# Xinjie-Q/Boosting-NeRV

Hardware: AMD Instinct MI355X
Metric: train frames/sec (higher is better)
Workload: dtype fp32; 1 GPU; NeRV-boost 1.5M (1489577 params, fc_dim 30) train step on a synthetic Bunny-shaped clip 132x3x720x1280: decoder fwd + Fusion10_freq + bwd + fused Adan; frames resident in HBM; global_batch=1, per_gpu_batch=1, parallelism=dp1, hipgraph=True, rccl_ranks=0, collective_in_graph=False

## Files before the change

### boosting_nerv_amd/csrc/abi.hip

```cpp
#include "common.h"
#include <string.h>

namespace { thread_local char g_err[512] = ""; }

int bnerv_set_error(int code, const char* fmt, ...) {
    va_list ap;
    va_start(ap, fmt);
    vsnprintf(g_err, sizeof(g_err), fmt, ap);
    va_end(ap);
    return code;
}

extern "C" int bnerv_abi_version(void) { return BNERV_ABI_VERSION; }
extern "C" const char* bnerv_last_error(void) { return g_err; }
extern "C" const char* bnerv_build_arch(void) { return "gfx950"; }

#include "sidejob.h"
#include <new>
#include <vector>

namespace {
__global__ __launch_bounds__(256) void side_flush_kernel(const SidePack sp) {
    __shared__ float red[256];
    side_slice<SidePack, true>(sp, blockIdx.x, red);
// ... 11 lines not shown
    j.out = out;
    j.out2 = out2;
    j.n_slabs = n_slabs;
    j.count = count;
    j.ncols = ncols;
    int lanes = 8;
    while (lanes < 128 && lanes * 16 < n_slabs) lanes *= 2;
    j.epb = 256 / lanes;
    j.slices = (count + j.epb - 1) / j.epb;
    return j;
}
}

void bnerv_side_push(bnerv_ctx* ctx, hipStream_t st, const void* src, int n_slabs, int count, int ncols, float* out, float* out2, const float* fold_scale, const float* fold_shift) {
    const SideJob j = make_job(src, n_slabs, count, ncols, out, out2, fold_scale, fold_shift);
    if (ctx) { ctx->queue.push_back(j); return; }
    SidePack sp;
    sp.j[0] = j;
    sp.n_jobs = 1;
    sp.n_slices = j.slices;
    hipLaunchKernelGGL(side_flush_kernel, dim3(sp.n_slices), dim3(256), 0, st, sp);
}

void bnerv_side_take(bnerv_ctx* ctx, SidePack* sp, int max_slices) {
    sp->n_jobs = 0;
    sp->n_slices = 0;
    if (!ctx) return;
    std::vector<SideJob>& q = ctx->queue;
    int n = 0;
    size_t i = 0;
    while (i < q.size() && n < SIDE_MAX_JOBS) {
        if (q[i].fs) { ++i; continue; }
        if (sp->n_slices + q[i].slices > max_slices) break;
        sp->j[n] = q[i];
        sp->n_slices += q[i].slices;
        ++n;
        q.erase(q.begin() + (long)i);
    }
    sp->n_jobs = n;
}

int bnerv_side_pending(const bnerv_ctx* ctx) { return ctx ? (int)ctx->queue.size() : 0; }

int bnerv_side_flush(bnerv_ctx* ctx, hipStream_t st) {
    while (ctx && !ctx->queue.empty()) {
        SideFlushPack sp;
        std::vector<SideJob>& q = ctx->queue;
        int n = 0;
        sp.n_slices = 0;
        while (n < (int)q.size() && n < SIDE_FLUSH_JOBS) {
            sp.j[n] = q[n];
            sp.start[n] = sp.n_slices;
            sp.n_slices += q[n].slices;
            ++n;
        }
        for (int k = n; k < SIDE_FLUSH_JOBS; ++k) sp.start[k] = 0x7fffffff;
// ... 57 lines not shown
```

### boosting_nerv_amd/csrc/sidejob.h

```cpp
#pragma once
#include "common.h"

constexpr int SIDE_MAX_JOBS = 4;

struct SideJob {
    const float* src;
    float* out;
    float* out2;
    int n_slabs, count, ncols;
    int epb;
    int slices;
    const float* fs;
    const float* ft;
};

struct SidePack {
    SideJob j[SIDE_MAX_JOBS];
    int n_jobs, n_slices;
};
constexpr int SIDE_FLUSH_JOBS = 32;
struct SideFlushPack {
    SideJob j[SIDE_FLUSH_JOBS];
    int n_jobs, n_slices;
    int start[SIDE_FLUSH_JOBS];
};

#include <vector>
struct bnerv_ctx {
    std::vector<SideJob> queue;
    void* scratch = nullptr;
    size_t scratch_bytes = 0;
    struct BfWPlan* wplan = nullptr;
};
void bnerv_wplan_free(bnerv_ctx* ctx);
void* bnerv_ctx_scratch(bnerv_ctx* ctx, size_t bytes, hipStream_t st);

void bnerv_side_push(bnerv_ctx* ctx, hipStream_t st, const void* src, int n_slabs, int count, int ncols, float* out, float* out2,
                     const float* fold_scale = nullptr, const float* fold_shift = nullptr);
void bnerv_side_take(bnerv_ctx* ctx, SidePack* sp, int max_slices);
int bnerv_side_flush(bnerv_ctx* ctx, hipStream_t st);
int bnerv_side_pending(const bnerv_ctx* ctx);

template <class Pack>
__device__ __forceinline__ int side_find_job(const Pack& sp, int* s) {
    int j = 0;
    while (j < sp.n_jobs - 1 && *s >= sp.j[j].slices) { *s -= sp.j[j].slices; ++j; }
    return j;
}
template <>
__device__ __forceinline__ int side_find_job<SideFlushPack>(const SideFlushPack& sp, int* s) {
    const int k = (int)(threadIdx.x & 63);
    const int st = k < sp.n_jobs ? sp.start[k < SIDE_FLUSH_JOBS ? k : 0] : 0x7fffffff;
    const unsigned long long m = __ballot(st <= *s);
    const int j = __popcll(m) - 1;
    *s -= __shfl(st, j, 64);
    return __builtin_amdgcn_readfirstlane(j);
}

template <class Pack, bool FOLD = false>
__device__ __forceinline__ void side_slice(const Pack& sp, int s, float* red) {
    const int j = side_find_job(sp, &s);
    const SideJob& job = sp.j[j];
// ... 70 lines not shown
```

### boosting_nerv_amd/csrc/wgrad.hip

```cpp
#include "common.h"
#include "sidejob.h"
#include "split16.h"
#include "conv4_body.h"
#include "convs_body.h"
#if defined(BNERV_TRACE) || defined(BNERV_TRACE_BW)
static __device__ unsigned long long g_trace_w[1024 * 4 * 8 * 8];
#endif
#ifdef BNERV_TRACE_BW
#define BTRACE(it_, slot) do { if (lane == 0 && blockIdx.x < 1024 && (unsigned)(it_) < 8u) g_trace_w[((blockIdx.x * 4 + wave) * 8 + (it_)) * 8 + (slot)] = __builtin_amdgcn_s_memtime(); } while (0)
#endif
#include "wgrad_bfw_body.h"
#include "route.h"
bool bnerv_stem_wgrad_ok(const bnerv_wgrad_desc& d);
int bnerv_stem_wgrad_launch(hipStream_t st, const bnerv_wgrad_desc& d);
bool bnerv_stem_pair_ok(const bnerv_conv_desc& c, const bnerv_wgrad_desc& d);
int bnerv_stem_pair_launch(hipStream_t st, const bnerv_conv_desc& c, const bnerv_wgrad_desc& d);
int bnerv_wgrad1x1_slabs(const bnerv_wgrad_desc& d);
int bnerv_wgrad1x1_launch(hipStream_t st, const bnerv_wgrad_desc& d);

namespace {
using namespace bnerv_wb;

constexpr int TH = 8, TW = 32;
constexpr int CSG = TH * TW + 2;
// ... 546 lines not shown

    int bbase[NTW];
#pragma unroll
    for (int nt = 0; nt < NTW; ++nt) {
        const int n = nt * 16 + li;
        int off;
        if (n < nW) {
            const int ci = n / G::T, tap = n - ci * G::T;
            off = ci * G::PLANE + (tap / KS) * G::RS + (tap % KS) + G::COL0;
        } else {
            off = (n == nW ? NPLL : NPLL + 1) * G::PLANE;
        }
        bbase[nt] = off + (2 * wave) * G::RS + kq;
    }
    const int abase = li * CSG + wave * 64 + kq;

    f32x4 acc[NTW];
#pragma unroll
    for (int n = 0; n < NTW; ++n) acc[n] = f32x4{0.f, 0.f, 0.f, 0.f};
    int aff_b = -1;
    if (has_work) {
        issue(it);
        if constexpr (AFF) { load_affine(it.b); aff_b = it.b; }
        commit(it);
    }
    WTRACE(7, 1);
    int wt = 0; (void)wt;
    for (; itx < r1; itx += nlb, ++wt) {
        WTRACE(wt, 0);
        const bool has_next = itx + nlb < r1;
        LTile nxt = it;
        if (has_next) nxt = advance(it);
        lds_barrier();
        WTRACE(wt, 1);
        const Pre pre = prep(nxt);
        WTRACE(wt, 2);
#pragma unroll
        for (int st = 0; st < 16; ++st) {
            if (has_next) {
#pragma unroll
                for (int p = 0; p < NPART; ++p)
                    if (p * 16 / NPART == st) issue_part(pre, p);
            }
            float bf[NTW];
            const float af = s_g[abase + st * 4];
#pragma unroll
            for (int n = 0; n < NTW; ++n) bf[n] = s_in[bbase[n] + ((st >> 3) * G::RS + (st & 7) * 4)];
#pragma unroll
            for (int n = 0; n < NTW; ++n) acc[n] = __builtin_amdgcn_mfma_f32_16x16x4f32(af, bf[n], acc[n], 0, 0, 0);
        }
        WTRACE(wt, 3);
        lds_barrier();
        WTRACE(wt, 5);
        if (has_next) {
            if constexpr (AFF) { if (nxt.b != aff_b) { load_affine(nxt.b); aff_b = nxt.b; } }
            commit(nxt);
        }
        WTRACE(wt, 6);
        it = nxt;
    }
    WTRACE(7, 2);

    __syncthreads();
    float* s_red = smem;
    constexpr int RW = NTW * 16, RSZ = 16 * RW;
#pragma unroll
    for (int n = 0; n < NTW; ++n)
#pragma unroll
        for (int r = 0; r < 4; ++r) s_red[wave * RSZ + (4 * kq + r) * RW + n * 16 + li] = acc[n][r];
    __syncthreads();
    float* slab = wa.slab + (size_t)vb * Cout * wa.ncols;
    for (int idx = tid; idx < RSZ; idx += 256) {
        const int row = idx / RW, col = idx - row * RW;
        if (row < Cout && col < wa.ncols)
            slab[(size_t)row * wa.ncols + col] = (s_red[idx] + s_red[RSZ + idx]) + (s_red[2 * RSZ + idx] + s_red[3 * RSZ + idx]);
    }
    WTRACE(7, 3);
    side_run_hosted(side, smem, vb, vgrid);
    WTRACE(7, 4);
}
template <int KS, int IN, int GM2>
__global__ __launch_bounds__(256, (KS == 3 ? 3 : 4)) void wgrad_lean_kernel(const WArgs wa, const int n_grows, const SidePack side) {
    wgrad_lean_body<KS, IN, GM2>(wa, n_grows, side, (int)blockIdx.x, (int)gridDim.x);
}
template <int EP, int WIN>
__global__ __launch_bounds__(256, 3) void conv_wgrad_pair_kernel(const bnerv_conv::KArgs ka, const WArgs wa, const int n_grows, const int n_conv, const SidePack side, const int pat) {
    if (n_conv < 0) {
        const int nr = -n_conv, xcd = (int)blockIdx.x & 7, slot = (int)blockIdx.x >> 3, vb = ((slot >> 1) << 3) + xcd;
        const int role = pat == 0 ? (slot & 1) : ((slot + (slot >> pat)) & 1);
        if (role == 0) {
            SidePack none;
            none.n_jobs = 0; none.n_slices = 0;
            bnerv_q4::conv_q4_body<BNERV_IN_PLAIN, EP>(ka, none, vb, nr);
        } else {
            wgrad_lean_body<3, WIN, 0>(wa, n_grows, side, vb, nr);
        }
        return;
    }
    if ((int)blockIdx.x < n_conv) {
        SidePack none;
        none.n_jobs = 0; none.n_slices = 0;
        bnerv_q4::conv_q4_body<BNERV_IN_PLAIN, EP>(ka, none, (int)blockIdx.x, n_conv);
    } else {
        wgrad_lean_body<3, WIN, 0>(wa, n_grows, side, (int)blockIdx.x - n_conv, (int)gridDim.x - n_conv);
    }
}

#include "pairf_body.h"
template <int EP, int WIN>
__global__ __launch_bounds__(256, 2) void pair_fused_kernel(const bnerv_conv::KArgs ka, const WArgs wa, const SidePack side) {
    pair_fused_body<EP, WIN>(ka, wa, side, (int)blockIdx.x, (int)gridDim.x);
}
template <int EP>
__global__ __launch_bounds__(256, 2) void pair_fold_kernel(const bnerv_conv::KArgs ka, const WArgs wa, const SidePack side) {
    pair_fold_body<EP>(ka, wa, side, (int)blockIdx.x, (int)gridDim.x);
}

constexpr size_t WLEAN_MAX_BYTES = 0x7ff00000;

template <class F>
int wlean_modes(const bnerv_wgrad_desc& d, F&& f) {
    const int in = d.in_mode, gm = d.g_mode;
    if (gm == BNERV_IN_TANHGRAD && in == BNERV_IN_PLAIN) return f(mode_c<BNERV_IN_PLAIN>{}, mode_c<2>{});
    if (gm == BNERV_IN_PLAIN || gm == BNERV_IN_UNSHUFFLE) {
        const bool pair = gm == BNERV_IN_UNSHUFFLE && d.g_s == 2;
        if (in == BNERV_IN_PLAIN) return pair ? f(mode_c<BNERV_IN_PLAIN>{}, mode_c<1>{}) : f(mode_c<BNERV_IN_PLAIN>{}, mode_c<0>{});
        if (d.k == 3 && !pair && in == BNERV_IN_AFFINE) return f(mode_c<BNERV_IN_AFFINE>{}, mode_c<0>{});
// ... 31 lines not shown
    const size_t lds_red = (size_t)4 * 16 * NTW * 16;
    return (lds_main > lds_red ? lds_main : lds_red) * sizeof(float);
}

template <int KS, int IN, int GM2>
int launch_wlean(hipStream_t st, const WArgs& wa) {
    const int n_grows = wa.d.Cout <= 12 ? 12 : 16;
    const size_t lds = wlean_lds_bytes<KS>(n_grows);
    SidePack side;
    bnerv_side_take(wa.d.ctx, &side, 2 * wlean_blocks(wa.d));
    hipLaunchKernelGGL((wgrad_lean_kernel<KS, IN, GM2>), dim3(wlean_blocks(wa.d)), dim3(256), lds, st, wa, n_grows, side);
    BNERV_LAUNCH_CHECK("wgrad_lean");
    return BNERV_OK;
}

static int launch_wlean_modes(hipStream_t st, const WArgs& wa) {
    return wlean_modes(wa.d, [&](auto in, auto gm2) {
        constexpr int IN = decltype(in)::value, GM2 = decltype(gm2)::value;
        if constexpr (IN == BNERV_IN_PLAIN) { if (wa.d.k == 1) return launch_wlean<1, IN, GM2>(st, wa); }
        return launch_wlean<3, IN, GM2>(st, wa);
    });
}

template <int MTW, int NTW>
size_t wgrad_wide_lds_bytes(int Cout) {
    const int g_rows = Cout < MTW * 16 ? Cout : MTW * 16;
    size_t fl = (size_t)g_rows * CSG + (size_t)(wgrad_npl<3, NTW>() + 2) * Geo<3>::PLANE + 64;
    if (fl < (size_t)MTW * 16 * CSG) fl = (size_t)MTW * 16 * CSG;
    if (fl < (size_t)MTW * 16 * NTW * 16) fl = (size_t)MTW * 16 * NTW * 16;
    return fl * sizeof(float);
}
template <int IN, int GM2, int MTW, int NTW>
__device__ __forceinline__ void wgrad_wide_body(const WArgs& wa, const int slots, const SidePack& side, const int vb, const int vgrid) {
    using G = Geo<3>;
    constexpr int NPL = wgrad_npl<3, NTW>();
    constexpr int NXSLOT = NPL * G::ROWS * G::SEGS;
    constexpr int NXS = (NXSLOT + 255) / 256;
    constexpr int NGS = (GM2 == 1) ? MTW * 2 : MTW * 4;
    constexpr bool GTWO = (GM2 == 1 || GM2 == 2);
    constexpr bool AFF = (IN == BNERV_IN_AFFINE || IN == BNERV_IN_GELU_AFFINE);
    constexpr int AFFN = 32;
    static_assert(NPL <= AFFN, "affine table too small");
    const bnerv_wgrad_desc& d = wa.d;
    extern __shared__ __attribute__((aligned(16))) float smem[];
    const int tid = threadIdx.x, lane = tid & 63;
    const int wave = __builtin_amdgcn_readfirstlane(tid >> 6);
    const int li = lane & 15, kq = lane >> 4;
    const int Cin = d.Cin, Cout = d.Cout, H = d.H, W = d.W;
    const int co_base = (int)(((vb >> 3) % (unsigned)(wa.n_ngroups * wa.n_mgroups)) / (unsigned)wa.n_ngroups) * MTW * 16;
    const int g_rows = min(MTW * 16, Cout - co_base);
    float* s_g = smem;
    float* s_in = smem + g_rows * CSG;
// ... 183 lines not shown
        int off;
        if (n < nW) {
            const int ci = n / G::T, tap = n - ci * G::T;
            off = (ci - ci_lo) * G::PLANE + (tap / 3) * G::RS + (tap % 3) + G::COL0;
        } else {
            off = (n == nW ? NPL : NPL + 1) * G::PLANE;
        }
        bbase[nt] = off + (2 * wave) * G::RS + kq;
    }
    const int abase = li * CSG + wave * 64 + kq;

    f32x4 acc[MTW][NTW];
#pragma unroll
    for (int m = 0; m < MTW; ++m)
#pragma unroll
        for (int n = 0; n < NTW; ++n) acc[m][n] = f32x4{0.f, 0.f, 0.f, 0.f};

    int aff_b = -1;
    if (has_work) {
        const Pre p0 = prep(it);
#pragma unroll
        for (int part = 0; part < NPART; ++part) issue_part(p0, part);
        if constexpr (AFF) { load_affine(it.b); aff_b = it.b; }
        commit(it);
    }
    for (; itx < r1; itx += slots) {
        const bool has_next = itx + slots < r1;
        LTile nxt = it;
        if (has_next) nxt = advance(it);
        lds_barrier();
        const Pre pre = prep(nxt);
        float af[2][MTW], bf[2][NTW];
#pragma unroll
        for (int m = 0; m < MTW; ++m) af[0][m] = s_g[abase + m * 16 * CSG];
#pragma unroll
        for (int n = 0; n < NTW; ++n) bf[0][n] = s_in[bbase[n]];
#pragma unroll
        for (int st = 0; st < 16; ++st) {
            if (has_next) {
#pragma unroll
                for (int part = 0; part < NPART; ++part)
                    if (part * 16 / NPART == st) issue_part(pre, part);
            }
            if (st < 15) {
#pragma unroll
                for (int m = 0; m < MTW; ++m) af[(st + 1) & 1][m] = s_g[abase + m * 16 * CSG + (st + 1) * 4];
#pragma unroll
                for (int n = 0; n < NTW; ++n) bf[(st + 1) & 1][n] = s_in[bbase[n] + (((st + 1) >> 3) * G::RS + ((st + 1) & 7) * 4)];
            }
#pragma unroll
            for (int m = 0; m < MTW; ++m)
#pragma unroll
                for (int n = 0; n < NTW; ++n) acc[m][n] = __builtin_amdgcn_mfma_f32_16x16x4f32(af[st & 1][m], bf[st & 1][n], acc[m][n], 0, 0, 0);
            __builtin_amdgcn_sched_barrier(0);
        }
        lds_barrier();
        if (has_next) {
            if constexpr (AFF) { if (nxt.b != aff_b) { load_affine(nxt.b); aff_b = nxt.b; } }
            commit(nxt);
        }
        it = nxt;
    }

    __syncthreads();
    float* s_red = smem;
    constexpr int RW = NTW * 16, RSZ = MTW * 16 * RW;
    for (int w = 0; w < 4; ++w) {
        if (wave == w) {
#pragma unroll
            for (int m = 0; m < MTW; ++m)
#pragma unroll
                for (int n = 0; n < NTW; ++n)
#pragma unroll
                    for (int r = 0; r < 4; ++r) {
                        float* qd = s_red + (m * 16 + 4 * kq + r) * RW + n * 16 + li;
                        *qd = (w == 0) ? acc[m][n][r] : *qd + acc[m][n][r];
                    }
        }
        __syncthreads();
    }
    float* slab = wa.slab + (size_t)(xcd * slots + slot) * Cout * wa.ncols;
    for (int idx = tid; idx < RSZ; idx += 256) {
        const int row = idx / RW, colq = idx - row * RW;
        const int col = n_base + colq;
        if (co_base + row < Cout && col < wa.ncols) slab[(size_t)(co_base + row) * wa.ncols + col] = s_red[idx];
    }
    side_run_hosted(side, smem, vb, vgrid);
}

struct WidePlan { int mtw, ntw, ngroups, mgroups, slots; };

static WidePlan wide_plan(const bnerv_wgrad_desc& d) {
    WidePlan p{0, 0, 0, 1, 0};
    const int ncols = d.Cin * 9 + 1, nt = cdiv(ncols, 16), mt = cdiv(d.Cout, 16);
    auto best = [&](int a, int b) { return cdiv(nt, a) * a < cdiv(nt, b) * b ? a : b; };
    if (mt == 1) { p.mtw = 1; p.ntw = 8; }
    else if (mt == 2) { p.mtw = 2; p.ntw = best(7, 9); }
    else if (mt == 3) { p.mtw = 3; p.ntw = best(6, 7); }
    else if (mt == 4) { p.mtw = 4; p.ntw = 4; }
    else { p.mtw = 3; p.ntw = best(6, 7); p.mgroups = cdiv(mt, 3); }
    p.ngroups = cdiv(nt, p.ntw);
    const int per_cu = p.mtw * p.ntw <= 8 ? 3 : 2;
    const int total_tiles = d.B * cdiv(d.H, TH) * cdiv(d.W, TW);
    int s = (256 * per_cu) / (8 * p.ngroups * p.mgroups);
    const int want = cdiv(total_tiles, 8);
    if (s > want) s = want;
    if (s < 1) s = 1;
    p.slots = s;
    return p;
}
// ... 259 lines not shown
    case BNERV_WGRAD_FAM_STEM: return bnerv_stem_wgrad_launch(st, d);
    case BNERV_WGRAD_FAM_GEMM1X1: rc = bnerv_wgrad1x1_launch(st, d); break;
    case BNERV_WGRAD_FAM_LEAN: rc = launch_wlean_modes(st, wa); break;
    case BNERV_WGRAD_FAM_WIDE_BF16: rc = launch_bw_modes(st, wa, r.bw); break;
    case BNERV_WGRAD_FAM_WIDE_F32: rc = launch_wide_modes(st, wa, r.wide); break;
    default: rc = d.k == 1 ? launch_modes<1>(st, wa, r.gen) : launch_modes<3>(st, wa, r.gen); break;
    }
    if (rc != BNERV_OK) return rc;
    const int count = d.Cout * wa.ncols;
    if (d.defer_finish && d.ctx) {
        bnerv_side_push(d.ctx, st, wa.slab, r.n_slabs, count, wa.ncols, d.dw, d.db);
        return BNERV_OK;
    }
    hipLaunchKernelGGL(wgrad_finish_kernel, dim3(cdiv(count, 32)), dim3(1024), 0, st, wa.slab, r.n_slabs, d.Cout, wa.ncols, d.dw, d.db);
    BNERV_LAUNCH_CHECK("wgrad_finish");
    return BNERV_OK;
}

namespace {
enum { Q4P_INTERLEAVED, Q4P_SHARED, Q4P_FOLD };
struct Q4PairPlan { int kind, grid, n_conv, n_w; };
constexpr int PAIR_MIX = 384, PAIR_PAT = 5;

Q4PairPlan q4_pair_plan(const bnerv_conv_desc& c, const bnerv_wgrad_desc& w) {
    Q4PairPlan p{};
    const int total_items = c.B * cdiv(c.W, bnerv_conv::TW) * cdiv(c.H, bnerv_conv::TH), ncols = w.Cin * 9 + 1;
    const int fused_env = switch_int("BNERV_PAIR_FUSED", -1);
    const bool red_ep = c.ep_mode == BNERV_EP_DGELU_SAVED || c.ep_mode == BNERV_EP_DSIN;
    const int fused_min = fused_env >= 0 ? fused_env : (red_ep ? 1024 : 0);
    if (fused_min > 0 && total_items >= fused_min && total_items >= 8 && c.x == w.g && c.Cin == w.Cout && c.Cout == w.Cin && c.B == w.B &&
        w.g_s == 1 && (w.g_mode == BNERV_IN_PLAIN || w.g_mode == BNERV_IN_UNSHUFFLE)) {
        p.kind = Q4P_SHARED;
        p.grid = p.n_w = total_items < 512 ? (total_items & ~7) : 512;
        const float* raw_aux = c.ep_mode == BNERV_EP_DSIN ? c.aux0 : c.aux1;
        if (red_ep && w.in_mode == BNERV_IN_AFFINE && !switch_off("BNERV_PAIR_FOLD") && c.B == 1 && raw_aux == w.x && w.scale && w.shift && aligned16(w.x) &&
            (size_t)p.grid * w.Cout * (ncols + 8) * sizeof(float) <= w.ws_bytes)
            p.kind = Q4P_FOLD;
        return p;
    }
    p.kind = Q4P_INTERLEAVED;
    p.n_conv = total_items < 768 ? total_items : 768;
    p.n_conv = (p.n_conv + 7) & ~7;
    p.n_w = wlean_blocks(w);
    p.grid = p.n_conv + p.n_w;
    if (total_items >= 2 * PAIR_MIX && p.n_w >= PAIR_MIX) {
        p.n_w = PAIR_MIX; p.n_conv = -PAIR_MIX; p.grid = 2 * PAIR_MIX;
// ... 20 lines not shown
            const size_t ldsf = pair_fused_lds_bytes();
            if (const int rc = dyn_lds<&pair_fused_kernel<EP, WIN>>(ldsf, "pair_fused")) return rc;
            const size_t ldsd = pair_fold_lds_bytes();
            if (const int rc = dyn_lds<&pair_fold_kernel<EP>>(ldsd, "pair_fold")) return rc;
            bnerv_side_take(wa.d.ctx, &side, 2 * p.n_w);
            hipLaunchKernelGGL((pair_fold_kernel<EP>), dim3(p.grid), dim3(256), ldsd, st, ka, wa, side);
            BNERV_LAUNCH_CHECK("pair_fold");
            return BNERV_OK;
        }
    }
    if (p.kind != Q4P_INTERLEAVED) {
        const size_t ldsf = pair_fused_lds_bytes();
        if (const int rc = dyn_lds<&pair_fused_kernel<EP, WIN>>(ldsf, "pair_fused")) return rc;
        bnerv_side_take(wa.d.ctx, &side, 2 * p.n_w);
        hipLaunchKernelGGL((pair_fused_kernel<EP, WIN>), dim3(p.grid), dim3(256), ldsf, st, ka, wa, side);
        BNERV_LAUNCH_CHECK("pair_fused");
        return BNERV_OK;
    }
    const int n_grows = wa.d.Cout <= 12 ? 12 : 16;
    size_t lds = bnerv_q4::q4_lds_bytes();
    const size_t lw = wlean_lds_bytes<3>(n_grows);
    if (lw > lds) lds = lw;
    if (const int rc = dyn_lds<&conv_wgrad_pair_kernel<EP, WIN>>(lds, "conv_wgrad_pair")) return rc;
    bnerv_side_take(wa.d.ctx, &side, 2 * p.n_w);
    hipLaunchKernelGGL((conv_wgrad_pair_kernel<EP, WIN>), dim3(p.grid), dim3(256), lds, st, ka, wa, n_grows, p.n_conv, side, PAIR_PAT);
    BNERV_LAUNCH_CHECK("conv_wgrad_pair");
    return BNERV_OK;
}

struct WideRoleArgs { int slots, ngn, ngm; };
template <int IN, int GM2, int MTW, int NTW>
struct WideRole {
    static __device__ __forceinline__ void run(const WArgs& wa, const WideRoleArgs& r, const SidePack& side, int vb, int vgrid) { wgrad_wide_body<IN, GM2, MTW, NTW>(wa, r.slots, side, vb, vgrid); }
    static size_t lds(const WArgs& wa) { return wgrad_wide_lds_bytes<MTW, NTW>(wa.d.Cout); }
};
template <int IN, int SP, int MTW, int GM2>
struct BfwRole {
    static __device__ __forceinline__ void run(const WArgs& wa, const WideRoleArgs& r, const SidePack& side, int vb, int vgrid) { wgrad_bfw_body<IN, SP, MTW, GM2>(wa, r.slots, r.ngn, r.ngm, side, vb, vgrid); }
    static size_t lds(const WArgs&) { return wgrad_bfw_lds_bytes<SP, MTW>(); }
};
template <class WR, int CIN, int CEP, int CNQ>
__global__ __launch_bounds__(256, 2) void small_pair_kernel(const bnerv_convs::SArgs sa, const WArgs wa, const WideRoleArgs r, const int n_c, const int n_c8,
                                                            const int c_tiles, const int c_groups, const SidePack side) {
    const int b = (int)blockIdx.x;
    if (b < n_c8) {
        if (b >= n_c) return;
        const int q = b / c_tiles;
        bnerv_convs::conv_small_body<CIN, CEP, CNQ>(sa, b - q * c_tiles, q % c_groups, q / c_groups);
    } else {
        WR::run(wa, r, side, b - n_c8, (int)gridDim.x - n_c8);
    }
}
template <class WR, int CIN, int CEP, int CNQ>
int launch_small_pair(hipStream_t st, const bnerv_convs::SArgs& sa, const WArgs& wa, const WideRoleArgs& r, int n_w) {
    size_t lds = bnerv_convs::convs_lds_bytes<CNQ>();
    const size_t lw = WR::lds(wa);
    if (lw > lds) lds = lw;
    if (const int rc = dyn_lds<&small_pair_kernel<WR, CIN, CEP, CNQ>>(lds, "small_pair")) return rc;
    const int c_tiles = sa.tiles_x * sa.tiles_y, c_groups = cdiv(sa.d.Cout, 16);
    const int n_c = c_tiles * c_groups * sa.d.B, n_c8 = (n_c + 7) & ~7;
    SidePack side;
    bnerv_side_take(wa.d.ctx, &side, 2 * n_w);
    hipLaunchKernelGGL((small_pair_kernel<WR, CIN, CEP, CNQ>), dim3(n_c8 + n_w), dim3(256), lds, st, sa, wa, r, n_c, n_c8, c_tiles, c_groups, side);
    BNERV_LAUNCH_CHECK("small_pair");
    return BNERV_OK;
}

template <class T> struct type_c { using type = T; };
template <class F>
int small_pair_modes(const bnerv_conv_desc& c, const bnerv_wgrad_desc& w, const WRoute& wr, F&& f) {
    const int cnq = bnerv_convs_nq(c);
    const bool up = w.g_s == 2 && w.in_mode == BNERV_IN_PLAIN && w.g_mode == BNERV_IN_UNSHUFFLE;
    const bool tat = w.g_s == 1 && w.in_mode == BNERV_IN_AFFINE && w.g_mode != BNERV_IN_TANHGRAD;
#define BNERV_SP(WR, I, E, Q) if (c.in_mode == I && c.ep_mode == E && cnq == Q) return f(type_c<WR>{}, mode_c<I>{}, mode_c<E>{}, mode_c<Q>{});
    if (wr.family == BNERV_WGRAD_FAM_WIDE_BF16 && split_wide_mode() == (int)SP_BF16X6) {
        if (up && wr.bw.mtw == 2) { using WR = BfwRole<BNERV_IN_PLAIN, SP_BF16X6, 2, 1>; BNERV_SP(WR, BNERV_IN_UNSHUFFLE, BNERV_EP_PLAIN, 8) BNERV_SP(WR, BNERV_IN_UNSHUFFLE, BNERV_EP_PLAIN, 16) }
        if (up && wr.bw.mtw == 3) { using WR = BfwRole<BNERV_IN_PLAIN, SP_BF16X6, 3, 1>; BNERV_SP(WR, BNERV_IN_UNSHUFFLE, BNERV_EP_PLAIN, 16) }
        if (tat && wr.bw.mtw == 2) { using WR = BfwRole<BNERV_IN_AFFINE, SP_BF16X6, 2, 0>; BNERV_SP(WR, BNERV_IN_PLAIN, BNERV_EP_DGELU_SAVED, 8) BNERV_SP(WR, BNERV_IN_PLAIN, BNERV_EP_DSIN, 8) }
    }
    if (wr.family == BNERV_WGRAD_FAM_WIDE_F32 && wr.wide.mtw == 1 && wr.wide.ntw == 8 && tat) {
        using WR = WideRole<BNERV_IN_AFFINE, 0, 1, 8>;
        BNERV_SP(WR, BNERV_IN_PLAIN, BNERV_EP_DGELU_SAVED, 4) BNERV_SP(WR, BNERV_IN_PLAIN, BNERV_EP_DSIN, 4)
    }
#undef BNERV_SP
    return -1;
}

bool small_pair_ok(const bnerv_conv_desc& c, int cvec, const bnerv_wgrad_desc& w, const WRoute& wr) {
    if (!bnerv_convs_ok(c, cvec) || bnerv_convs_nq(c) == 24) return false;
    if (c.ep_mode == BNERV_EP_PLAIN && bnerv_conv_splitk_ws_bytes(&c) != 0) return false;
    if (!(w.k == 3 && w.B == c.B && w.H == c.H && w.W == c.W && w.defer_finish && w.ctx && w.ctx == c.ctx)) return false;
    return small_pair_modes(c, w, wr, [](auto...) { return 0; }) == 0;
}

int small_pair_launch(hipStream_t st, const bnerv_conv_desc& c, const WArgs& wa, const WRoute& wr) {
    const bnerv_convs::SArgs sa = bnerv_convs_sargs(c);
    const bool bf = wr.family == BNERV_WGRAD_FAM_WIDE_BF16;
    const WideRoleArgs r = bf ? WideRoleArgs{wr.bw.slots, wr.bw.ngroups_n, wr.bw.ngroups_m} : WideRoleArgs{wr.wide.slots, 0, 0};
    const int n_w = bf ? 8 * wr.bw.slots * wr.bw.ngroups_n * wr.bw.ngroups_m : 8 * wr.wide.slots * wr.wide.ngroups * wr.wide.mgroups;
    return small_pair_modes(c, wa.d, wr, [&](auto role, auto in, auto ep, auto nq) {
        return launch_small_pair<typename decltype(role)::type, decltype(in)::value, decltype(ep)::value, decltype(nq)::value>(st, sa, wa, r, n_w);
    });
}
}

constexpr int HB_KMAX = 4, HB_CMAX = 16;
struct HeadBwdArgs { const float* g; const float* img; const float* x; const float* w; float* dx; float* slab; int B, K, C, transposed; size_t HW; int nq; };
template <int K, int C>
__global__ __launch_bounds__(256) void head1x1_bwd_kernel(const HeadBwdArgs a) {
    __shared__ float s_w[HB_KMAX * HB_CMAX];
    __shared__ float s_red[4][HB_KMAX * (HB_CMAX + 1)];
    const int tid = threadIdx.x, lane = tid & 63, wave = tid >> 6;
    if (tid < K * C) {
        const int k = tid / C, c = tid - k * C;
        s_w[k * HB_CMAX + c] = a.transposed ? a.w[k * C + c] : a.w[c * K + k];
    }
    if (lane < K * (C + 1)) s_red[wave][(lane / (C + 1)) * (HB_CMAX + 1) + lane % (C + 1)] = 0.f;
    __syncthreads();
    const int total = a.B * a.nq;
    const int rounds = (total + (int)gridDim.x * 256 - 1) / ((int)gridDim.x * 256);
#pragma unroll 1
    for (int it = 0; it < rounds; ++it) {
        const int q = (it * (int)gridDim.x + (int)blockIdx.x) * 256 + tid;
        const bool live = q < total;
// ... 198 lines not shown
```

### boosting_nerv_amd/csrc/wgrad_bfw_body.h

```cpp
#pragma once
#include "common.h"
#include "sidejob.h"
#include "split16.h"
#ifndef BTRACE
#define BTRACE(it_, slot) do {} while (0)
#endif

namespace bnerv_wb {

struct WArgs {
    bnerv_wgrad_desc d;
    float* slab;
    int tiles_x, tiles_y, n_mgroups, n_ngroups, ncols;
    int vec;
};

typedef int i32x4 __attribute__((ext_vector_type(4)));
constexpr unsigned OOB = 0x80000000u;

__device__ __forceinline__ __amdgpu_buffer_rsrc_t make_rsrc(const float* p, unsigned shift_bytes, unsigned bytes) {
    return __builtin_amdgcn_make_buffer_rsrc(reinterpret_cast<void*>(reinterpret_cast<uintptr_t>(p) - shift_bytes), 0, (int)bytes, 0x00020000);
}
__device__ __forceinline__ f32x4 bload(__amdgpu_buffer_rsrc_t r, unsigned voff, unsigned soff) {
    return __builtin_bit_cast(f32x4, __builtin_amdgcn_raw_buffer_load_b128(r, (int)voff, (int)soff, 0));
}

struct LTile { int b, ty, tx; };

constexpr int BW_TH = 4, BW_NTW = 8, BW_NPL = (BW_NTW * 16 + 7) / 9 + 1;
constexpr int BW_ROW = 64, BW_PLANE = 6 * BW_ROW + 32, BW_COPY = BW_NPL * BW_PLANE + 192, BW_CONST = 4 * BW_ROW;
constexpr int BW_PIECE = 3 * BW_COPY + 2 * BW_CONST;

template <int IN, int SP, int MTW, int GM2>
__device__ __forceinline__ void wgrad_bfw_body(const WArgs& wa, const int slots, const int ngroups_n, const int ngroups_m, const SidePack& side, const int vb, const int vgrid) {
    constexpr int NS = Split<SP>::NS;
    constexpr bool AFF = (IN == BNERV_IN_AFFINE);
    constexpr int PIECE = BW_PIECE;
    const bnerv_wgrad_desc& d = wa.d;
    extern __shared__ __attribute__((aligned(16))) float smem[];
    char* s_a = reinterpret_cast<char*>(smem);
    float* s_aff = reinterpret_cast<float*>(s_a + NS * PIECE);
    const int tid = threadIdx.x, lane = tid & 63;
    const int wave = __builtin_amdgcn_readfirstlane(tid >> 6);
    const int li = lane & 15, kq = lane >> 4;
    const int Cin = d.Cin, Cout = d.Cout, H = d.H, W = d.W;
    const int nW = Cin * 9;
    const int tiles_x = (W + 31) >> 5, tiles_y = (H + BW_TH - 1) / BW_TH;

    const int ngroups = ngroups_n * ngroups_m;
    const int xcd = vb & 7, q = vb >> 3;
// ... 180 lines not shown
#pragma unroll
    for (int m = 0; m < MTW; ++m)
#pragma unroll
        for (int n = 0; n < BW_NTW; ++n) acc[m][n] = f32x4{0.f, 0.f, 0.f, 0.f};

    int itx = r0 + slot;
    LTile it{0, 0, 0};
    auto decode = [&](int i) __attribute__((always_inline)) {
        LTile t;
        const int tiles = tiles_x * tiles_y;
        t.b = i / tiles;
        const int rem = i - t.b * tiles;
        t.ty = rem / tiles_x;
        t.tx = rem - t.ty * tiles_x;
        return t;
    };
    int aff_b = -1;
    if (itx < r1) {
        it = decode(itx);
        issue_loads(it);
        if constexpr (AFF) { load_affine(it.b); aff_b = it.b; }
        lds_barrier();
        if constexpr (AFF) fetch_affine();
        store_x(tile_interior(it));
    }
    int bt = -3;
    for (; itx < r1; itx += slots, ++bt) {
        BTRACE(bt, 0);
        const bool has_next = itx + slots < r1;
        LTile nxt = it;
        if (has_next) nxt = decode(itx + slots);
        u32x4 afr[MTW][NS];
        auto split_g = [&](auto mc) __attribute__((always_inline)) {
            constexpr int m = decltype(mc)::value;
            if constexpr (m < MTW) {
                float x[8] = {ga[m][0].x, ga[m][0].y, ga[m][0].z, ga[m][0].w, ga[m][1].x, ga[m][1].y, ga[m][1].z, ga[m][1].w};
                if constexpr (GM2 == 1) {
                    const bool odd = li & 1;
                    const float k0 = odd ? x[1] : x[0], k1 = odd ? x[3] : x[2], k2 = odd ? x[5] : x[4], k3 = odd ? x[7] : x[6];
                    const float s0 = odd ? x[0] : x[1], s1 = odd ? x[2] : x[3], s2 = odd ? x[4] : x[5], s3 = odd ? x[6] : x[7];
                    const float r0 = __builtin_bit_cast(float, __builtin_amdgcn_update_dpp(0, __builtin_bit_cast(int, s0), 0xB1, 0xF, 0xF, false));
                    const float r1 = __builtin_bit_cast(float, __builtin_amdgcn_update_dpp(0, __builtin_bit_cast(int, s1), 0xB1, 0xF, 0xF, false));
                    const float r2 = __builtin_bit_cast(float, __builtin_amdgcn_update_dpp(0, __builtin_bit_cast(int, s2), 0xB1, 0xF, 0xF, false));
                    const float r3 = __builtin_bit_cast(float, __builtin_amdgcn_update_dpp(0, __builtin_bit_cast(int, s3), 0xB1, 0xF, 0xF, false));
                    x[0] = odd ? r0 : k0; x[1] = odd ? r1 : k1; x[2] = odd ? r2 : k2; x[3] = odd ? r3 : k3;
                    x[4] = odd ? k0 : r0; x[5] = odd ? k1 : r1; x[6] = odd ? k2 : r2; x[7] = odd ? k3 : r3;
                }
                split8<SP, 8>(x, afr[m]);
            }
        };
        split_g(std::integral_constant<int, 0>{});
        split_g(std::integral_constant<int, 1>{});
        split_g(std::integral_constant<int, 2>{});
        BTRACE(bt, 1);
        if (has_next) issue_loads(nxt);
        BTRACE(bt, 2);
        lds_barrier();
        BTRACE(bt, 3);
#pragma unroll
        for (int nt = 0; nt < BW_NTW; ++nt) {
            u32x4 bfr[NS];
#pragma unroll
            for (int p = 0; p < NS; ++p) bfr[p] = *reinterpret_cast<const u32x4*>(s_a + p * PIECE + bbase[nt]);
#define BNERV_BW_PROD(pa, pb) _Pragma("unroll") for (int m = 0; m < MTW; ++m) acc[m][nt] = mfma16<SP>(afr[m][pa], bfr[pb], acc[m][nt]);
            if constexpr (NS == 3) {
                BNERV_BW_PROD(2, 0)
                BNERV_BW_PROD(0, 2)
                BNERV_BW_PROD(1, 1)
            }
            BNERV_BW_PROD(1, 0)
            BNERV_BW_PROD(0, 1)
            BNERV_BW_PROD(0, 0)
#undef BNERV_BW_PROD
        }
        BTRACE(bt, 4);
        lds_barrier();
        BTRACE(bt, 5);
        if (has_next) {
            if constexpr (AFF) { if (nxt.b != aff_b) { load_affine(nxt.b); lds_barrier(); fetch_affine(); aff_b = nxt.b; } }
            if (tile_interior(nxt)) store_x(true);
            else store_x(false);
        }
        BTRACE(bt, 6);
        it = nxt;
    }

    __syncthreads();
    float* s_red = smem;
    constexpr int RW = BW_NTW * 16, RSZ = MTW * 16 * RW;
    for (int w = 0; w < 4; ++w) {
        if (wave == w) {
#pragma unroll
            for (int m = 0; m < MTW; ++m)
#pragma unroll
                for (int n = 0; n < BW_NTW; ++n)
#pragma unroll
                    for (int r = 0; r < 4; ++r) {
                        float* qd = s_red + (m * 16 + 4 * kq + r) * RW + n * 16 + li;
                        *qd = (w == 0) ? acc[m][n][r] : *qd + acc[m][n][r];
                    }
        }
        __syncthreads();
    }
    float* slab = wa.slab + (size_t)(xcd * slots + slot) * Cout * wa.ncols;
    for (int idx = tid; idx < RSZ; idx += 256) {
        const int row = idx / RW, colq = idx - row * RW;
        const int col = n_base + colq;
        if (co_base + row < Cout && col < wa.ncols) slab[(size_t)(co_base + row) * wa.ncols + col] = s_red[idx];
    }
    side_run_hosted(side, smem, vb, vgrid);
}

struct BwPlan { int mtw, ngroups_n, ngroups_m, slots; };
template <int SP, int MTW>
constexpr size_t wgrad_bfw_lds_bytes() {
    const size_t acc = (size_t)Split<SP>::NS * BW_PIECE + 2 * BW_NPL * sizeof(float), red = (size_t)MTW * 16 * BW_NTW * 16 * sizeof(float);
    return acc > red ? acc : red;
}

}
```

Before: 687.2 frames/s.

## Cut wgrad reduction barriers and host side jobs on conv blocks in pair kernels

The serial four-wave LDS reduction in the wide and bf16 wgrad epilogues becomes a single-barrier scheme. Each wave writes its accumulators to a private LDS region and the final loop sums all four, chunked by M for the bf16 path. This trades more LDS for fewer __syncthreads. The pair kernels can now hand deferred side-reduction jobs to conv blocks instead of wgrad blocks, and side_take skips oversized jobs rather than stopping at them. Compile-time ablation switches (BNERV_WABL, BNERV_WRED4) are added and default to off.

```diff
diff --git a/boosting_nerv_amd/csrc/abi.hip b/boosting_nerv_amd/csrc/abi.hip
--- a/boosting_nerv_amd/csrc/abi.hip
+++ b/boosting_nerv_amd/csrc/abi.hip
@@ -57,7 +57,7 @@
     hipLaunchKernelGGL(side_flush_kernel, dim3(sp.n_slices), dim3(256), 0, st, sp);
 }
 
-void bnerv_side_take(bnerv_ctx* ctx, SidePack* sp, int max_slices) {
+void bnerv_side_take(bnerv_ctx* ctx, SidePack* sp, int max_slices, bool step_over) {
     sp->n_jobs = 0;
     sp->n_slices = 0;
     if (!ctx) return;
@@ -66,7 +66,11 @@
     size_t i = 0;
     while (i < q.size() && n < SIDE_MAX_JOBS) {
         if (q[i].fs) { ++i; continue; }
-        if (sp->n_slices + q[i].slices > max_slices) break;
+        if (sp->n_slices + q[i].slices > max_slices) {
+            if (!step_over) break;
+            ++i;
+            continue;
+        }
         sp->j[n] = q[i];
         sp->n_slices += q[i].slices;
         ++n;
diff --git a/boosting_nerv_amd/csrc/sidejob.h b/boosting_nerv_amd/csrc/sidejob.h
--- a/boosting_nerv_amd/csrc/sidejob.h
+++ b/boosting_nerv_amd/csrc/sidejob.h
@@ -37,7 +37,7 @@
 
 void bnerv_side_push(bnerv_ctx* ctx, hipStream_t st, const void* src, int n_slabs, int count, int ncols, float* out, float* out2,
                      const float* fold_scale = nullptr, const float* fold_shift = nullptr);
-void bnerv_side_take(bnerv_ctx* ctx, SidePack* sp, int max_slices);
+void bnerv_side_take(bnerv_ctx* ctx, SidePack* sp, int max_slices, bool step_over = false);
 int bnerv_side_flush(bnerv_ctx* ctx, hipStream_t st);
 int bnerv_side_pending(const bnerv_ctx* ctx);
 
diff --git a/boosting_nerv_amd/csrc/wgrad.hip b/boosting_nerv_amd/csrc/wgrad.hip
--- a/boosting_nerv_amd/csrc/wgrad.hip
+++ b/boosting_nerv_amd/csrc/wgrad.hip
@@ -592,7 +592,7 @@
     if (has_work) {
         issue(it);
         if constexpr (AFF) { load_affine(it.b); aff_b = it.b; }
-        commit(it);
+        if (!((BNERV_WABL & 4) && d.B > 0)) commit(it);
     }
     WTRACE(7, 1);
     int wt = 0; (void)wt;
@@ -605,6 +605,7 @@
         WTRACE(wt, 1);
         const Pre pre = prep(nxt);
         WTRACE(wt, 2);
+        if (!((BNERV_WABL & 8) && d.B > 0))
 #pragma unroll
         for (int st = 0; st < 16; ++st) {
             if (has_next) {
@@ -624,7 +625,7 @@
         WTRACE(wt, 5);
         if (has_next) {
             if constexpr (AFF) { if (nxt.b != aff_b) { load_affine(nxt.b); aff_b = nxt.b; } }
-            commit(nxt);
+            if (!((BNERV_WABL & 4) && d.B > 0)) commit(nxt);
         }
         WTRACE(wt, 6);
         it = nxt;
@@ -634,6 +635,7 @@
     __syncthreads();
     float* s_red = smem;
     constexpr int RW = NTW * 16, RSZ = 16 * RW;
+    if (!((BNERV_WABL & 2) && d.B > 0)) {
 #pragma unroll
     for (int n = 0; n < NTW; ++n)
 #pragma unroll
@@ -645,8 +647,9 @@
         if (row < Cout && col < wa.ncols)
             slab[(size_t)row * wa.ncols + col] = (s_red[idx] + s_red[RSZ + idx]) + (s_red[2 * RSZ + idx] + s_red[3 * RSZ + idx]);
     }
+    }
     WTRACE(7, 3);
-    side_run_hosted(side, smem, vb, vgrid);
+    if (!(BNERV_WABL & 1)) side_run_hosted(side, smem, vb, vgrid);
     WTRACE(7, 4);
 }
 template <int KS, int IN, int GM2>
@@ -654,25 +657,24 @@
     wgrad_lean_body<KS, IN, GM2>(wa, n_grows, side, (int)blockIdx.x, (int)gridDim.x);
 }
 template <int EP, int WIN>
-__global__ __launch_bounds__(256, 3) void conv_wgrad_pair_kernel(const bnerv_conv::KArgs ka, const WArgs wa, const int n_grows, const int n_conv, const SidePack side, const int pat) {
+__global__ __launch_bounds__(256, 3) void conv_wgrad_pair_kernel(const bnerv_conv::KArgs ka, const WArgs wa, const int n_grows, const int n_conv, const SidePack side_c,
+                                                                 const SidePack side_w, const int pat) {
     if (n_conv < 0) {
         const int nr = -n_conv, xcd = (int)blockIdx.x & 7, slot = (int)blockIdx.x >> 3, vb = ((slot >> 1) << 3) + xcd;
         const int role = pat == 0 ? (slot & 1) : ((slot + (slot >> pat)) & 1);
         if (role == 0) {
-            SidePack none;
-            none.n_jobs = 0; none.n_slices = 0;
-            bnerv_q4::conv_q4_body<BNERV_IN_PLAIN, EP>(ka, none, vb, nr);
+            bnerv_q4::conv_q4_body<BNERV_IN_PLAIN, EP>(ka, side_c, vb, nr);
         } else {
-            wgrad_lean_body<3, WIN, 0>(wa, n_grows, side, vb, nr);
+            if (BNERV_WABL & 16) return;
+            wgrad_lean_body<3, WIN, 0>(wa, n_grows, side_w, vb, nr);
         }
         return;
     }
     if ((int)blockIdx.x < n_conv) {
-        SidePack none;
-        none.n_jobs = 0; none.n_slices = 0;
-        bnerv_q4::conv_q4_body<BNERV_IN_PLAIN, EP>(ka, none, (int)blockIdx.x, n_conv);
+        bnerv_q4::conv_q4_body<BNERV_IN_PLAIN, EP>(ka, side_c, (int)blockIdx.x, n_conv);
     } else {
-        wgrad_lean_body<3, WIN, 0>(wa, n_grows, side, (int)blockIdx.x - n_conv, (int)gridDim.x - n_conv);
+        if (BNERV_WABL & 16) return;
+        wgrad_lean_body<3, WIN, 0>(wa, n_grows, side_w, (int)blockIdx.x - n_conv, (int)gridDim.x - n_conv);
     }
 }
 
@@ -750,12 +752,14 @@
     });
 }
 
+template <int MTW, int NTW> constexpr bool wide_one_barrier() { return MTW * NTW <= 8 && !BNERV_WRED4; }
 template <int MTW, int NTW>
 size_t wgrad_wide_lds_bytes(int Cout) {
     const int g_rows = Cout < MTW * 16 ? Cout : MTW * 16;
     size_t fl = (size_t)g_rows * CSG + (size_t)(wgrad_npl<3, NTW>() + 2) * Geo<3>::PLANE + 64;
     if (fl < (size_t)MTW * 16 * CSG) fl = (size_t)MTW * 16 * CSG;
-    if (fl < (size_t)MTW * 16 * NTW * 16) fl = (size_t)MTW * 16 * NTW * 16;
+    const size_t red = (size_t)(wide_one_barrier<MTW, NTW>() ? 4 : 1) * MTW * 16 * NTW * 16;
+    if (fl < red) fl = red;
     return fl * sizeof(float);
 }
 template <int IN, int GM2, int MTW, int NTW>
@@ -985,7 +989,7 @@
 #pragma unroll
         for (int part = 0; part < NPART; ++part) issue_part(p0, part);
         if constexpr (AFF) { load_affine(it.b); aff_b = it.b; }
-        commit(it);
+        if (!((BNERV_WABL & 4) && d.B > 0)) commit(it);
     }
     for (; itx < r1; itx += slots) {
         const bool has_next = itx + slots < r1;
@@ -998,6 +1002,7 @@
         for (int m = 0; m < MTW; ++m) af[0][m] = s_g[abase + m * 16 * CSG];
 #pragma unroll
         for (int n = 0; n < NTW; ++n) bf[0][n] = s_in[bbase[n]];
+        if (!((BNERV_WABL & 8) && d.B > 0))
 #pragma unroll
         for (int st = 0; st < 16; ++st) {
             if (has_next) {
@@ -1020,7 +1025,7 @@
         lds_barrier();
         if (has_next) {
             if constexpr (AFF) { if (nxt.b != aff_b) { load_affine(nxt.b); aff_b = nxt.b; } }
-            commit(nxt);
+            if (!((BNERV_WABL & 4) && d.B > 0)) commit(nxt);
         }
         it = nxt;
     }
@@ -1028,6 +1033,17 @@
     __syncthreads();
     float* s_red = smem;
     constexpr int RW = NTW * 16, RSZ = MTW * 16 * RW;
+    constexpr bool ONEB = wide_one_barrier<MTW, NTW>();
+    if (!((BNERV_WABL & 2) && d.B > 0)) {
+    if constexpr (ONEB) {
+#pragma unroll
+        for (int m = 0; m < MTW; ++m)
+#pragma unroll
+            for (int n = 0; n < NTW; ++n)
+#pragma unroll
+                for (int r = 0; r < 4; ++r) s_red[wave * RSZ + (m * 16 + 4 * kq + r) * RW + n * 16 + li] = acc[m][n][r];
+        __syncthreads();
+    } else
     for (int w = 0; w < 4; ++w) {
         if (wave == w) {
 #pragma unroll
@@ -1046,9 +1062,12 @@
     for (int idx = tid; idx < RSZ; idx += 256) {
         const int row = idx / RW, colq = idx - row * RW;
         const int col = n_base + colq;
-        if (co_base + row < Cout && col < wa.ncols) slab[(size_t)(co_base + row) * wa.ncols + col] = s_red[idx];
-    }
-    side_run_hosted(side, smem, vb, vgrid);
+        float v = s_red[idx];
+        if constexpr (ONEB) v = ((v + s_red[RSZ + idx]) + s_red[2 * RSZ + idx]) + s_red[3 * RSZ + idx];
+        if (co_base + row < Cout && col < wa.ncols) slab[(size_t)(co_base + row) * wa.ncols + col] = v;
+    }
+    }
+    if (!(BNERV_WABL & 1)) side_run_hosted(side, smem, vb, vgrid);
 }
 
 struct WidePlan { int mtw, ntw, ngroups, mgroups, slots; };
@@ -1354,6 +1373,8 @@
 struct Q4PairPlan { int kind, grid, n_conv, n_w; };
 constexpr int PAIR_MIX = 384, PAIR_PAT = 5;
 
+inline bool pair_hosts_on_conv(int items, int blocks) { return items <= blocks; }
+
 Q4PairPlan q4_pair_plan(const bnerv_conv_desc& c, const bnerv_wgrad_desc& w) {
     Q4PairPlan p{};
     const int total_items = c.B * cdiv(c.W, bnerv_conv::TW) * cdiv(c.H, bnerv_conv::TH), ncols = w.Cin * 9 + 1;
@@ -1420,8 +1441,11 @@
     const size_t lw = wlean_lds_bytes<3>(n_grows);
     if (lw > lds) lds = lw;
     if (const int rc = dyn_lds<&conv_wgrad_pair_kernel<EP, WIN>>(lds, "conv_wgrad_pair")) return rc;
-    bnerv_side_take(wa.d.ctx, &side, 2 * p.n_w);
-    hipLaunchKernelGGL((conv_wgrad_pair_kernel<EP, WIN>), dim3(p.grid), dim3(256), lds, st, ka, wa, n_grows, p.n_conv, side, PAIR_PAT);
+    SidePack none;
+    none.n_jobs = 0; none.n_slices = 0;
+    const bool on_conv = p.n_conv > 0 && pair_hosts_on_conv(ka.total_items, p.n_conv);
+    bnerv_side_take(wa.d.ctx, &side, 2 * (on_conv ? p.n_conv : p.n_w), true);
+    hipLaunchKernelGGL((conv_wgrad_pair_kernel<EP, WIN>), dim3(p.grid), dim3(256), lds, st, ka, wa, n_grows, p.n_conv, on_conv ? side : none, on_conv ? none : side, PAIR_PAT);
     BNERV_LAUNCH_CHECK("conv_wgrad_pair");
     return BNERV_OK;
 }
@@ -1439,27 +1463,34 @@
 };
 template <class WR, int CIN, int CEP, int CNQ>
 __global__ __launch_bounds__(256, 2) void small_pair_kernel(const bnerv_convs::SArgs sa, const WArgs wa, const WideRoleArgs r, const int n_c, const int n_c8,
-                                                            const int c_tiles, const int c_groups, const SidePack side) {
+                                                            const int c_tiles, const int c_groups, const SidePack side_c, const SidePack side_w) {
+    extern __shared__ __attribute__((aligned(16))) float smem[];
     const int b = (int)blockIdx.x;
     if (b < n_c8) {
-        if (b >= n_c) return;
-        const int q = b / c_tiles;
-        bnerv_convs::conv_small_body<CIN, CEP, CNQ>(sa, b - q * c_tiles, q % c_groups, q / c_groups);
+        if (b < n_c) {
+            const int q = b / c_tiles;
+            bnerv_convs::conv_small_body<CIN, CEP, CNQ>(sa, b - q * c_tiles, q % c_groups, q / c_groups);
+        }
+        if (!(BNERV_WABL & 1)) side_run_hosted(side_c, smem, b, n_c8);
     } else {
-        WR::run(wa, r, side, b - n_c8, (int)gridDim.x - n_c8);
+        if (BNERV_WABL & 16) return;
+        WR::run(wa, r, side_w, b - n_c8, (int)gridDim.x - n_c8);
     }
 }
 template <class WR, int CIN, int CEP, int CNQ>
-int launch_small_pair(hipStream_t st, const bnerv_convs::SArgs& sa, const WArgs& wa, const WideRoleArgs& r, int n_w) {
+int launch_small_pair(hipStream_t st, const bnerv_convs::SArgs& sa, const WArgs& wa, const WideRoleArgs& r, int n_w, int w_tiles) {
     size_t lds = bnerv_convs::convs_lds_bytes<CNQ>();
     const size_t lw = WR::lds(wa);
     if (lw > lds) lds = lw;
     if (const int rc = dyn_lds<&small_pair_kernel<WR, CIN, CEP, CNQ>>(lds, "small_pair")) return rc;
     const int c_tiles = sa.tiles_x * sa.tiles_y, c_groups = cdiv(sa.d.Cout, 16);
     const int n_c = c_tiles * c_groups * sa.d.B, n_c8 = (n_c + 7) & ~7;
-    SidePack side;
-    bnerv_side_take(wa.d.ctx, &side, 2 * n_w);
-    hipLaunchKernelGGL((small_pair_kernel<WR, CIN, CEP, CNQ>), dim3(n_c8 + n_w), dim3(256), lds, st, sa, wa, r, n_c, n_c8, c_tiles, c_groups, side);
+    SidePack side, none;
+    none.n_jobs = 0; none.n_slices = 0;
+    const bool on_conv = pair_hosts_on_conv(w_tiles, 8 * r.slots);
+    bnerv_side_take(wa.d.ctx, &side, 2 * (on_conv ? n_c8 : n_w), true);
+    hipLaunchKernelGGL((small_pair_kernel<WR, CIN, CEP, CNQ>), dim3(n_c8 + n_w), dim3(256), lds, st, sa, wa, r, n_c, n_c8, c_tiles, c_groups, on_conv ? side : none,
+                       on_conv ? none : side);
     BNERV_LAUNCH_CHECK("small_pair");
     return BNERV_OK;
 }
@@ -1496,8 +1527,9 @@
     const bool bf = wr.family == BNERV_WGRAD_FAM_WIDE_BF16;
     const WideRoleArgs r = bf ? WideRoleArgs{wr.bw.slots, wr.bw.ngroups_n, wr.bw.ngroups_m} : WideRoleArgs{wr.wide.slots, 0, 0};
     const int n_w = bf ? 8 * wr.bw.slots * wr.bw.ngroups_n * wr.bw.ngroups_m : 8 * wr.wide.slots * wr.wide.ngroups * wr.wide.mgroups;
+    const int w_tiles = wa.d.B * cdiv(wa.d.H, bf ? BW_TH : TH) * cdiv(wa.d.W, TW);
     return small_pair_modes(c, wa.d, wr, [&](auto role, auto in, auto ep, auto nq) {
-        return launch_small_pair<typename decltype(role)::type, decltype(in)::value, decltype(ep)::value, decltype(nq)::value>(st, sa, wa, r, n_w);
+        return launch_small_pair<typename decltype(role)::type, decltype(in)::value, decltype(ep)::value, decltype(nq)::value>(st, sa, wa, r, n_w, w_tiles);
     });
 }
 }
diff --git a/boosting_nerv_amd/csrc/wgrad_bfw_body.h b/boosting_nerv_amd/csrc/wgrad_bfw_body.h
--- a/boosting_nerv_amd/csrc/wgrad_bfw_body.h
+++ b/boosting_nerv_amd/csrc/wgrad_bfw_body.h
@@ -5,6 +5,9 @@
 #ifndef BTRACE
 #define BTRACE(it_, slot) do {} while (0)
 #endif
+#ifndef BNERV_WABL
+#define BNERV_WABL 0
+#endif
 
 namespace bnerv_wb {
 
@@ -26,6 +29,10 @@
 }
 
 struct LTile { int b, ty, tx; };
+#ifndef BNERV_WRED4
+#define BNERV_WRED4 0
+#endif
+template <int MTW> constexpr int bfw_red_chunk() { return BNERV_WRED4 ? 0 : (MTW < 2 ? MTW : 2); }
 
 constexpr int BW_TH = 4, BW_NTW = 8, BW_NPL = (BW_NTW * 16 + 7) / 9 + 1;
 constexpr int BW_ROW = 64, BW_PLANE = 6 * BW_ROW + 32, BW_COPY = BW_NPL * BW_PLANE + 192, BW_CONST = 4 * BW_ROW;
@@ -252,7 +259,7 @@
         if constexpr (AFF) { load_affine(it.b); aff_b = it.b; }
         lds_barrier();
         if constexpr (AFF) fetch_affine();
-        store_x(tile_interior(it));
+        if (!((BNERV_WABL & 4) && d.B > 0)) store_x(tile_interior(it));
     }
     int bt = -3;
     for (; itx < r1; itx += slots, ++bt) {
@@ -287,6 +294,7 @@
         BTRACE(bt, 2);
         lds_barrier();
         BTRACE(bt, 3);
+        if (!((BNERV_WABL & 8) && d.B > 0))
 #pragma unroll
         for (int nt = 0; nt < BW_NTW; ++nt) {
             u32x4 bfr[NS];
@@ -308,7 +316,8 @@
         BTRACE(bt, 5);
         if (has_next) {
             if constexpr (AFF) { if (nxt.b != aff_b) { load_affine(nxt.b); lds_barrier(); fetch_affine(); aff_b = nxt.b; } }
-            if (tile_interior(nxt)) store_x(true);
+            if ((BNERV_WABL & 4) && d.B > 0) {}
+            else if (tile_interior(nxt)) store_x(true);
             else store_x(false);
         }
         BTRACE(bt, 6);
@@ -318,6 +327,33 @@
     __syncthreads();
     float* s_red = smem;
     constexpr int RW = BW_NTW * 16, RSZ = MTW * 16 * RW;
+    constexpr int MCH = bfw_red_chunk<MTW>();
+    float* slab = wa.slab + (size_t)(xcd * slots + slot) * Cout * wa.ncols;
+    if (!((BNERV_WABL & 2) && d.B > 0)) {
+    if constexpr (MCH > 0) {
+        constexpr int CSZ = MCH * 16 * RW;
+#pragma unroll
+        for (int m0 = 0; m0 < MTW; m0 += MCH) {
+            const int mc = MTW - m0 < MCH ? MTW - m0 : MCH;
+            if (m0 > 0) __syncthreads();
+#pragma unroll
+            for (int m = 0; m < MCH; ++m)
+                if (m < mc) {
+#pragma unroll
+                    for (int n = 0; n < BW_NTW; ++n)
+#pragma unroll
+                        for (int r = 0; r < 4; ++r)
+                            s_red[wave * CSZ + (m * 16 + 4 * kq + r) * RW + n * 16 + li] = acc[m0 + m < MTW ? m0 + m : 0][n][r];
+                }
+            __syncthreads();
+            for (int idx = tid; idx < mc * 16 * RW; idx += 256) {
+                const int row = idx / RW, colq = idx - row * RW;
+                const int col = n_base + colq, co = co_base + m0 * 16 + row;
+                const float v = ((s_red[idx] + s_red[CSZ + idx]) + s_red[2 * CSZ + idx]) + s_red[3 * CSZ + idx];
+                if (co < Cout && col < wa.ncols) slab[(size_t)co * wa.ncols + col] = v;
+            }
+        }
+    } else {
     for (int w = 0; w < 4; ++w) {
         if (wave == w) {
 #pragma unroll
@@ -332,19 +368,20 @@
         }
         __syncthreads();
     }
-    float* slab = wa.slab + (size_t)(xcd * slots + slot) * Cout * wa.ncols;
     for (int idx = tid; idx < RSZ; idx += 256) {
         const int row = idx / RW, colq = idx - row * RW;
         const int col = n_base + colq;
         if (co_base + row < Cout && col < wa.ncols) slab[(size_t)(co_base + row) * wa.ncols + col] = s_red[idx];
     }
-    side_run_hosted(side, smem, vb, vgrid);
+    }
+    }
+    if (!(BNERV_WABL & 1)) side_run_hosted(side, smem, vb, vgrid);
 }
 
 struct BwPlan { int mtw, ngroups_n, ngroups_m, slots; };
 template <int SP, int MTW>
 constexpr size_t wgrad_bfw_lds_bytes() {
-    const size_t acc = (size_t)Split<SP>::NS * BW_PIECE + 2 * BW_NPL * sizeof(float), red = (size_t)MTW * 16 * BW_NTW * 16 * sizeof(float);
+    const size_t acc = (size_t)Split<SP>::NS * BW_PIECE + 2 * BW_NPL * sizeof(float), red = (size_t)(bfw_red_chunk<MTW>() ? 4 * bfw_red_chunk<MTW>() : MTW) * 16 * BW_NTW * 16 * sizeof(float);
     return acc > red ? acc : red;
 }
 
```

After: 698.0 frames/s, median of 6. 1.02x the previous value.
